# leejeongho3214/LightHand

Hardware: AMD Instinct MI355X
Metric: images/sec/GPU (256×256, bs=64) train+infer; EPE/AUC parity (higher is better)
Workload: dtype bf16; 1 GPU; SimpleBaseline-ResNet50 256x256 training step (fwd + JointsMSELoss + argmax decode + bwd + Adam), batch 64/GPU, 21 joints, random init (seed 9001), hipGraph replay; global_batch=64, parallelism=dp1

## Files before the change

include/lighthand_hip.h:

```cpp
#ifndef LIGHTHAND_HIP_H
#define LIGHTHAND_HIP_H

#include <stddef.h>
#include <stdint.h>

#ifdef __cplusplus
extern "C" {
#endif

typedef enum { LH_F32 = 0, LH_BF16 = 1, LH_F16 = 2 } lh_dtype;

typedef enum {
    LH_OK = 0,
    LH_ERR_ARG = -1,
    LH_ERR_HIP = -2,
    LH_ERR_UNSUPPORTED = -3
} lh_status;

int lh_version(void);
const char* lh_last_error(void);
int lh_dtype_size(int dtype);

int lh_image_to_nhwc4(const float* nchw, void* out, int n, int h, int w, int pad, int wp,
                      int dtype, void* stream);
// ... 74 lines not shown
    const float* mean2;
    const float* invstd2;
    float* partial2;
} lh_bn_bwd_gate;
int lh_igemm_gated_rows(const lh_igemm_desc* d, int dtype, int nterms);
int lh_igemm_gated(const lh_igemm_desc* d, const void* in, const void* wpack, void* out, const void* addend, const void* addend_mask,
                   const lh_bn_bwd_gate* gate, int dtype, void* stream);
int lh_igemm_phases_rows(const lh_igemm_desc* const* descs, int nphase, int dtype);
int lh_igemm_phases(const lh_igemm_desc* const* descs, int nphase, const void* in, const void* const* wpacks,
                    void* out, const void* addend, const void* addend_mask, const float* bias, const float* scale,
                    const float* shift, float* stats, int dtype, void* stream);
typedef struct {
    const void* w;
    size_t w_row_bytes;
    const float* bias;
    float* out;
    int n_out;
} lh_head;
int lh_igemm_phases_head(const lh_igemm_desc* const* descs, int nphase, const void* in, const void* const* wpacks,
                         const float* scale, const float* shift, const lh_head* head, int dtype, void* stream);
int lh_igemm_tile(const lh_igemm_desc* d, int dtype, int* bm, int* bp, int* ring);
int lh_igemm_config(const lh_igemm_desc* d, int dtype, int* cfg5);
int lh_igemm_candidates(const lh_igemm_desc* d, int dtype, int* cfgs, int max);
int lh_wgrad_rowfold(const lh_igemm_desc* d, int rows, const void* x, const void* dy, int dy_pix_stride,
                     int n_out, float* slab, int dtype, void* stream);
int lh_wgrad_tile(const lh_igemm_desc* d, int n_out, int n_in, int dtype, int* bo, int* bi, int* nsplit, int* ring);
int lh_wgrad_candidates(const lh_igemm_desc* d, int n_out, int n_in, int dtype, int* out, int max);
typedef struct {
    const lh_igemm_desc* d; const void* in; const void* wpack; void* out; const void* addend; const void* addend_mask;
    const float* bias; const float* scale; const float* shift; float* stats;
} lh_igemm_call;
int lh_igemm_multi(const lh_igemm_call* calls, int n, int dtype, void* stream);
int lh_igemm_stats_rows(const lh_igemm_desc* d, int dtype);

size_t lh_wgrad_slab_bytes(const lh_igemm_desc* d, int n_out, int n_in, int dtype);
int lh_wgrad(const lh_igemm_desc* d, const void* x, const void* dy, int dy_pix_stride,
             int n_out, int n_in, float* slab, int dtype, void* stream);
int lh_wgrad_reduce(const lh_igemm_desc* d, const float* slab, float* grad, int n_out, int n_in,
                    long so, long si, long sr, long ss, const int* taps_rs, int accumulate,
                    int dtype, void* stream);
size_t lh_wgrad_workspace_bytes(const lh_igemm_desc* d, int n_out, int n_in, int dtype);
typedef struct {
    const lh_igemm_desc* d; int rows; const void* x; const void* dy; int dy_pix_stride, n_out, n_in; void* workspace; float* grad;
    long so, si, sr, ss; const int* taps_rs; int accumulate;
} lh_wgrad_call;
int lh_wgrad_fused_multi(const lh_wgrad_call* calls, int n, int dtype, void* stream);
int lh_wgrad_fused(const lh_igemm_desc* d, int rows, const void* x, const void* dy, int dy_pix_stride, int n_out, int n_in,
                   void* workspace, float* grad, long so, long si, long sr, long ss, const int* taps_rs, int accumulate,
                   int dtype, void* stream);
typedef struct {
    int bo, bi, kps, depth;
    int n_problems, n_fold;
    int n_items, n_fold_items;
    int fold_lds, target_stages, nsplit_max;
    int run_parts;
    size_t off_items, off_fold_args, off_fold_items, table_bytes, workspace_bytes;
} lh_wgrad_table_info;
int lh_wgrad_table_build(const lh_wgrad_call* calls, int n, int dtype, const int* cfg4, int target_stages, void* workspace,
                         void* host_blob, size_t host_bytes, lh_wgrad_table_info* info);
int lh_wgrad_table_run(const void* table, const lh_wgrad_table_info* info, int dtype, void* stream);


int lh_bn_stats(const void* y, int m, int c, float* stats, int* rows_out, int dtype, void* stream);
int lh_bn_stats_rows(int m, int c);
size_t lh_bn_stats_slab_bytes(int rows, int c);
int lh_bn_finalize(const float* stats, int rows, int count, int c, const float* gamma,
// ... 147 lines not shown
```

lighthand_amd/_lib.py:

```python
import ctypes as C
import os

_HERE = os.path.dirname(os.path.abspath(__file__))
LIB_PATH = os.environ.get("LH_LIB_PATH") or os.path.join(_HERE, "liblighthand_hip.so")

LH_F32, LH_BF16, LH_F16 = 0, 1, 2


class LightHandError(RuntimeError):
    pass


class IgemmDesc(C.Structure):
    _fields_ = [("n", C.c_int), ("hi", C.c_int), ("wi", C.c_int), ("in_pix_stride", C.c_int),
                ("k_run", C.c_int), ("ho", C.c_int), ("wo", C.c_int), ("sh", C.c_int), ("sw", C.c_int),
                ("cout", C.c_int), ("OH", C.c_int), ("OW", C.c_int), ("osh", C.c_int), ("osw", C.c_int),
                ("ooh", C.c_int), ("oow", C.c_int), ("out_pix_stride", C.c_int), ("ntaps", C.c_int),
                ("relu", C.c_int), ("dh", C.c_byte * 64), ("dw", C.c_byte * 64), ("cfg", C.c_int * 8)]


class BnFinalizeCall(C.Structure):
    _fields_ = [("stats", C.c_void_p), ("rows", C.c_int), ("count", C.c_int), ("c", C.c_int), ("gamma", C.c_void_p), ("beta", C.c_void_p),
                ("running_mean", C.c_void_p), ("running_var", C.c_void_p), ("num_batches_tracked", C.c_void_p), ("momentum", C.c_float),
                ("eps", C.c_float), ("scale", C.c_void_p), ("shift", C.c_void_p), ("save_mean", C.c_void_p), ("save_invstd", C.c_void_p)]
# ... 69 lines not shown
                ("packs", PackOut * 5)]


_P, _I, _L, _F, _SZ = C.c_void_p, C.c_int, C.c_long, C.c_float, C.c_size_t

SIGNATURES = {
    "lh_version": (_I, []),
    "lh_last_error": (C.c_char_p, []),
    "lh_dtype_size": (_I, [_I]),
    "lh_image_to_nhwc4": (_I, [_P, _P, _I, _I, _I, _I, _I, _I, _P]),
    "lh_image_u8_to_nhwc4": (_I, [_P, _P, _I, _I, _I, _I, _I, _I, _I, C.POINTER(C.c_float), C.POINTER(C.c_float), _I, _P]),
    "lh_image_jitter_workspace_bytes": (_SZ, [_I]),
    "lh_image_u8_jitter_to_nhwc4": (_I, [_P, _P, _I, _I, _I, _I, _I, _I, _I, C.POINTER(C.c_float), C.POINTER(C.c_float), _P, _P, _P, _I, _P]),
    "lh_image_u8_warp_to_nhwc4": (_I, [_P, _P, _I, _I, _I, _I, _I, _I, _I, C.POINTER(C.c_float), C.POINTER(C.c_float), _P, _P, _P, _P, _I, _P]),
    "lh_affine_points": (_I, [_P, _I, _P, _P, _I, _I, _I, _P]),
    "lh_nhwc4_mirror": (_I, [_P, _I, _I, _I, _I, _I, _I, _P]),
    "lh_nhwc_to_nchw_f32": (_I, [_P, _P, _I, _I, _I, _I, _I, _I, _P]),
    "lh_nchw_f32_to_nhwc": (_I, [_P, _P, _I, _I, _I, _I, _I, _I, _P]),
    "lh_pack_weight": (_I, [_P, _P, C.POINTER(_SZ), _I, _I, _L, _L, _L, _L, _I, C.POINTER(_I), _I, _P]),
    "lh_pack_chunk_elems": (_I, []),
    "lh_pack_weights_multi": (_I, [_P, _P, _P, _I, _I, _P]),
    "lh_pack_weights_tiled": (_I, [_P, _P, _P, _P, _I, _I, _I, _P]),
    "lh_igemm": (_I, [C.POINTER(IgemmDesc), _P, _P, _P, _P, _P, _P, _P, _P, _P, _I, _P]),
    "lh_igemm_multi": (_I, [C.POINTER(IgemmCall), _I, _I, _P]),
    "lh_igemm_phases_rows": (_I, [C.POINTER(C.POINTER(IgemmDesc)), _I, _I]),
    "lh_igemm_phases": (_I, [C.POINTER(C.POINTER(IgemmDesc)), _I, _P, C.POINTER(C.c_void_p), _P, _P, _P, _P, _P, _P, _P, _I, _P]),
    "lh_igemm_phases_head": (_I, [C.POINTER(C.POINTER(IgemmDesc)), _I, _P, C.POINTER(C.c_void_p), _P, _P, C.POINTER(Head), _I, _P]),
    "lh_igemm_tile": (_I, [C.POINTER(IgemmDesc), _I, C.POINTER(_I), C.POINTER(_I), C.POINTER(_I)]),
    "lh_igemm_config": (_I, [C.POINTER(IgemmDesc), _I, C.POINTER(_I)]),
    "lh_igemm_candidates": (_I, [C.POINTER(IgemmDesc), _I, C.POINTER(_I), _I]),
    "lh_wgrad_tile": (_I, [C.POINTER(IgemmDesc), _I, _I, _I, C.POINTER(_I), C.POINTER(_I), C.POINTER(_I), C.POINTER(_I)]),
    "lh_wgrad_candidates": (_I, [C.POINTER(IgemmDesc), _I, _I, _I, C.POINTER(_I), _I]),
    "lh_igemm_stats_rows": (_I, [C.POINTER(IgemmDesc), _I]),
    "lh_igemm_gated_rows": (_I, [C.POINTER(IgemmDesc), _I, _I]),
    "lh_igemm_gated": (_I, [C.POINTER(IgemmDesc), _P, _P, _P, _P, _P, C.POINTER(BnBwdGate), _I, _P]),
    "lh_wgrad_slab_bytes": (_SZ, [C.POINTER(IgemmDesc), _I, _I, _I]),
    "lh_wgrad": (_I, [C.POINTER(IgemmDesc), _P, _P, _I, _I, _I, _P, _I, _P]),
    "lh_wgrad_rowfold": (_I, [C.POINTER(IgemmDesc), _I, _P, _P, _I, _I, _P, _I, _P]),
    "lh_wgrad_workspace_bytes": (_SZ, [C.POINTER(IgemmDesc), _I, _I, _I]),
    "lh_wgrad_fused": (_I, [C.POINTER(IgemmDesc), _I, _P, _P, _I, _I, _I, _P, _P, _L, _L, _L, _L, C.POINTER(_I), _I, _I, _P]),
    "lh_wgrad_fused_multi": (_I, [C.POINTER(WgradCall), _I, _I, _P]),
    "lh_wgrad_table_build": (_I, [C.POINTER(WgradCall), _I, _I, C.POINTER(_I), _I, _P, _P, _SZ, C.POINTER(WgradTableInfo)]),
    "lh_wgrad_table_run": (_I, [_P, C.POINTER(WgradTableInfo), _I, _P]),
    "lh_wgrad_reduce": (_I, [C.POINTER(IgemmDesc), _P, _P, _I, _I, _L, _L, _L, _L, C.POINTER(_I), _I, _I, _P]),
    "lh_bn_stats": (_I, [_P, _I, _I, _P, C.POINTER(_I), _I, _P]),
    "lh_bn_stats_rows": (_I, [_I, _I]),
    "lh_bn_stats_slab_bytes": (_SZ, [_I, _I]),
    "lh_bn_finalize": (_I, [_P, _I, _I, _I, _P, _P, _P, _P, _P, _F, _F, _P, _P, _P, _P, _P]),
    "lh_bn_finalize_multi": (_I, [C.POINTER(BnFinalizeCall), _I, _P]),
    "lh_bn_eval_affine": (_I, [_P, _P, _P, _P, _F, _I, _P, _P, _P]),
    "lh_fuse_fwd": (_I, [C.POINTER(FuseDesc), _P, _I, _I, _I, _I, _I, _P]),
    "lh_fuse_fwd_multi": (_I, [C.POINTER(FuseFwdCall), _I, _I, _P]),
    "lh_fuse_bwd_multi": (_I, [C.POINTER(FuseBwdCall), _I, _I, _P]),
    "lh_fuse_bwd_workspace_bytes": (_SZ, [_I, _I, _I, _I]),
    "lh_fuse_bwd": (_I, [C.POINTER(FuseBwdDesc), _I, _I, _I, _I, _P, _I, _P]),
    "lh_stem_pool": (_I, [_P, _I, _I, _I, _P, _P, _P, _P, _P, _I, _I, _I, _I, _P]),
    "lh_bottleneck_infer": (_I, [C.POINTER(BottleneckDesc), _P, _P, _P, _P, _P, _P, _P, _P, _P, _P, _P, _P, _I, _P]),
    "lh_stem_conv_rows": (_I, [_I, _I, _I]),
    "lh_stem_conv": (_I, [_P, _I, _I, _I, _P, _P, _P, _I, _I, _I, _P]),
    "lh_maxpool3x3s2_fwd": (_I, [_P, _P, _P, _I, _I, _I, _I, _I, _P]),
    "lh_maxpool3x3s2_bwd": (_I, [_P, _P, _P, _I, _I, _I, _I, _I, _P]),
    "lh_bn_relu_maxpool3x3s2_fwd": (_I, [_P, _P, _P, _P, _P, _I, _I, _I, _I, _I, _P]),
    "lh_maxpool3x3s2_bwd_gated_rows": (_I, [_I, _I, _I, _I, _I]),
    "lh_maxpool3x3s2_bwd_gated": (_I, [_P, _P, _P, C.POINTER(BnBwdGate), _I, _I, _I, _I, _I, _P]),
    "lh_gaussian_target": (_I, [_P, _I, _P, _I, _P, _I, _I, _I, _P]),
    "lh_gaussian_target_alt": (_I, [_P, _I, _P, _I, _P, _I, _I, _I, _P]),
# ... 65 lines not shown
```

lighthand_amd/csrc/igemm.hip:

```cpp
#include "common.h"
#include <cstring>
#include <algorithm>
#include <stdlib.h>

#include "igemm_args.h"
#include "multi.h"
#include "igemm_ring_cfgs.h"

template <typename T> struct Mma;
template <> struct Mma<bf16> {
    static __device__ __forceinline__ void run(const uint4& a, const uint4& b, f32x4& c) {
        c = __builtin_amdgcn_mfma_f32_16x16x32_bf16(__builtin_bit_cast(bf16x8, a),
                                                   __builtin_bit_cast(bf16x8, b), c, 0, 0, 0);
    }
};
template <> struct Mma<f16> {
    static __device__ __forceinline__ void run(const uint4& a, const uint4& b, f32x4& c) {
        c = __builtin_amdgcn_mfma_f32_16x16x32_f16(__builtin_bit_cast(f16x8, a),
                                                  __builtin_bit_cast(f16x8, b), c, 0, 0, 0);
    }
};
template <> struct Mma<float> {
    static __device__ __forceinline__ void run(const uint4& a, const uint4& b, f32x4& c) {
        const f32x4 fa = __builtin_bit_cast(f32x4, a), fb = __builtin_bit_cast(f32x4, b);
// ... 334 lines not shown
        LH_REQUIRE(gate->x && gate->mean && gate->invstd && gate->partial && (gate->mask || (gate->scale && gate->shift)),
                   "lh_igemm_gated: null pointer in the gate (the sign of the activation comes from scale + shift or from mask)");
        LH_REQUIRE(!bias && !scale && !d->relu && !phases && !head, "lh_igemm_gated: a data gradient carries no bias / affine / ReLU / phases");
        LH_REQUIRE(!gate->mask || d->out_pix_stride == d->cout, "lh_igemm_gated: gate.mask needs a dense output (mask bits index 16-byte chunks)");
        a.gx = (const unsigned char*)gate->x; a.gmean = gate->mean; a.ginv = gate->invstd; a.gscale = gate->scale; a.gshift = gate->shift;
        a.gmask = (const unsigned char*)gate->mask;
        a.stats = gate->partial;
        if (gate->x2) {
            LH_REQUIRE(gate->mask && gate->mean2 && gate->invstd2 && gate->partial2, "lh_igemm_gated: a second BatchNorm term (x2) needs mask, mean2, invstd2, partial2");
            a.gx2 = (const unsigned char*)gate->x2; a.gmean2 = gate->mean2; a.ginv2 = gate->invstd2; a.stats2 = gate->partial2;
        }
    }
    a.n = d->n; a.hi = d->hi; a.wi = d->wi; a.in_pix_stride = d->in_pix_stride; a.k_run = d->k_run;
    a.kspt = (d->k_run * es + 63) / 64;
    a.kpad = (d->k_run * es + 127) / 128 * (128 / es);
    a.ho = d->ho; a.wo = d->wo; a.M = d->n * d->ho * d->wo; a.sh = d->sh; a.sw = d->sw; a.cout = d->cout;
    a.OH = d->OH; a.OW = d->OW; a.osh = d->osh; a.osw = d->osw; a.ooh = d->ooh; a.oow = d->oow;
    a.out_pix_stride = d->out_pix_stride; a.ntaps = d->ntaps; a.relu = d->relu;
    for (int i = 0; i < 64; ++i) { a.dh[i] = d->dh[i]; a.dw[i] = d->dw[i]; }
    int bm, bp;
    RingCfg rc_;
    const bool ring = lh_ring_supported(d, dtype);
    if (ring) {
        const int rc = lh_ring_resolve(d, dtype, &rc_);
        if (rc) return rc;
        bm = rc_.bm; bp = rc_.bp;
    } else {
        pick_tile(d, dtype, &bm, &bp);
    }
    hipStream_t s = (hipStream_t)stream;
    a.tw = 1; a.dh0 = a.dhs = a.dw0 = a.dws = 0;
    a.xcd = 1;
    a.nphase = 1; a.phase_blocks = 0;
    LH_REQUIRE(!(ring && (rc_.depth == 1 || rc_.depth == 100) && (phases || head)), "lh_igemm_phases: the persistent kernels take single launches only");
    if (phases) {
        LH_REQUIRE(ring, "lh_igemm_phases: the form is not supported by the LDS-DMA kernel");
        a.nphase = phases->n;
        a.phase_blocks = ceil_div(a.M, bp) * ceil_div(a.cout, bm);
        for (int i = 0; i < phases->n; ++i) {
            const lh_igemm_desc* q = phases->descs[i];
            a.ph_w[i] = (const unsigned char*)phases->wpacks[i];
            a.ph_ntaps[i] = q->ntaps; a.ph_tw[i] = 1; a.ph_dh0[i] = a.ph_dhs[i] = a.ph_dw0[i] = a.ph_dws[i] = 0;
            if (q->ntaps > 0)
                LH_REQUIRE(lh_tap_grid(q, &a.ph_tw[i], &a.ph_dh0[i], &a.ph_dhs[i], &a.ph_dw0[i], &a.ph_dws[i]) && a.ph_w[i],
                           "lh_igemm_phases: phase %d has an irregular tap list or no weights", i);
            a.ph_ooh[i] = q->ooh; a.ph_oow[i] = q->oow;
            a.ph_row0[i] = i * ceil_div(a.M, bp);
        }
    }
    if (head) {
        LH_REQUIRE(head->w && head->out && head->n_out >= 1 && head->n_out <= 32 && head->w_row_bytes >= d->cout * es,
                   "lh_igemm_phases_head: bad head (1..32 output channels, K-major weight rows)");
        LH_REQUIRE(ring && es == 2 && bm == 256 && bp == 256 && d->cout <= 256 && !addend && !stats,
                   "lh_igemm_phases_head: needs the 256 x 256 tile of the LDS-DMA kernel (cfg), a 16-bit type, <= 256 channels, no addend / statistics");
        a.head_w = (const unsigned char*)head->w; a.head_bias = head->bias; a.head_out = head->out;
        a.head_j = head->n_out; a.head_wstride = (int)head->w_row_bytes;
    }
    if (prep_args) {
        LH_REQUIRE(ring && ((rc_.depth >= 2 && rc_.depth < LH_WIDE_DEPTH) || rc_.depth == 100),
                   "lh_igemm_multi: problem does not run on the LDS-DMA ring kernel or the direct 3x3 kernel (its cfg must name a tiled or the direct configuration)");
        if (rc_.depth == 100) {
            a.pw_cb = (d->cout + 63) / 64;
            a.pw_g = lh_d3_rows(d);
        } else {
            lh_tap_grid(d, &a.tw, &a.dh0, &a.dhs, &a.dw0, &a.dws);
            a.kspt = (d->k_run * es + rc_.kb - 1) / rc_.kb;
// ... 145 lines not shown
```

lighthand_amd/csrc/igemm_args.h:

```cpp
#pragma once
#include "common.h"

struct IgemmArgs {
    const unsigned char* in;
    const unsigned char* w;
    unsigned char* out;
    const unsigned char* addend;
    const unsigned char* addend_mask;
    const unsigned char* zero;
    unsigned char* dump;
    const float* bias;
    const float* scale;
    const float* shift;
    float* stats;
    const unsigned char* gx;
    const float* gmean;
    const float* ginv;
    const float* gscale;
    const float* gshift;
    const unsigned char* gmask;
    const unsigned char* gx2;
    const float* gmean2;
    const float* ginv2;
    float* stats2;
    const unsigned char* head_w;
    const float* head_bias;
    float* head_out;
    int head_j, head_wstride;
    int n, hi, wi, in_pix_stride, k_run, kspt, kpad;
    int ho, wo, M, sh, sw, cout;
    int OH, OW, osh, osw, ooh, oow, out_pix_stride;
    int ntaps, relu;
    int nphase, phase_blocks;
    const unsigned char* ph_w[4];
    int ph_ntaps[4], ph_tw[4], ph_dh0[4], ph_dhs[4], ph_dw0[4], ph_dws[4], ph_ooh[4], ph_oow[4], ph_row0[4];
    int xcd;
    int pw_g, pw_cb;
    int tw, dh0, dhs, dw0, dws;
    signed char dh[64];
    signed char dw[64];
};

struct RingCfg {
    int bm, bp, depth, kb;
};

static inline int lh_pw_lds_bytes(int bm, int kc, int pt, int gate = 0) {
    return bm * kc * 2 + 4 * pt * 16 * (64 * 2 + 8) + (2 + 2 * gate) * bm * 4;
}

static inline void lh_pw_grid(int bm, int kc, int pt, long M, int cout, int occ, int* G, int* CB) {
    const int cb = (cout + bm - 1) / bm;
    const long ntile = (M + pt * 16 - 1) / (pt * 16);
    long g = 256L * occ / cb / 8 * 8;
    const long need = ((ntile + 3) / 4 + 7) / 8 * 8;
    if (g > need) g = need;
    if (g < 8) g = 8;
    *G = (int)g;
    *CB = cb;
}


bool lh_ring_supported(const lh_igemm_desc* d, int dtype);
bool lh_tap_grid(const lh_igemm_desc* d, int* tw, int* dh0, int* dhs, int* dw0, int* dws);
int lh_ring_resolve(const lh_igemm_desc* d, int dtype, RingCfg* out);
void lh_ring_default_cfg(const lh_igemm_desc* d, int dtype, RingCfg* out);
int lh_ring_candidates(const lh_igemm_desc* d, int dtype, int* out, int max);
int lh_igemm_ring_launch(const IgemmArgs& a, const RingCfg& c, int dtype, hipStream_t s);
template <typename A> struct LhMulti;
int lh_igemm_ring_multi_launch(LhMulti<IgemmArgs>& m, const RingCfg& c, int dtype, hipStream_t s);
bool lh_pw_supported(const lh_igemm_desc* d, int dtype);
// ... 5 lines not shown
```

lighthand_amd/csrc/igemm_epilogue.h:

```cpp
#pragma once
#include "common.h"
#include "igemm_args.h"

#ifndef LH_ABL
#define LH_ABL 0
#endif

template <typename T, int BM, int BP, bool HEAD> constexpr int lh_epi_lds_bytes() {
    return BP * (BM * (int)sizeof(T) + 8) + (HEAD ? 32 * (BM * (int)sizeof(T) + 16) : 0) + 3 * BM * 4;
}

template <int BM, int NT>
__device__ __forceinline__ void igemm_epilogue_consts(const IgemmArgs& p, float* cst, int c0, int tid) {
    const int cmax = p.cout - 1;
    for (int c = tid; c < BM; c += NT) {
        const int gc = c0 + c, gk = gc < cmax ? gc : cmax;
        const bool ok = gc < p.cout;
        const float b = p.bias ? p.bias[gk] : 0.f, sc = p.scale ? p.scale[gk] : 1.f, sh = p.scale ? p.shift[gk] : 0.f;
        float bv = (p.bias && ok) ? b : 0.f, sv = 1.f;
        if (p.scale) {
            sv = ok ? sc : 1.f;
            bv = bv * sv + (ok ? sh : 0.f);
        }
        cst[c] = sv;
// ... 37 lines not shown
            b4 = *reinterpret_cast<const float4*>(cst + BM + col);
        }
        const float sv[4] = {s4.x, s4.y, s4.z, s4.w}, bv[4] = {b4.x, b4.y, b4.z, b4.w};
#pragma unroll
        for (int j = 0; j < PT; ++j) {
            const int pr = wp * TP + j * 16 + pl;
            T* dst = reinterpret_cast<T*>(smem + pr * RS + col * ES);
            if constexpr (ES == 4) {
                reinterpret_cast<float2*>(dst)[0] = float2{acc[i][j][0] * sv[0] + bv[0], acc[i][j][1] * sv[1] + bv[1]};
                reinterpret_cast<float2*>(dst)[1] = float2{acc[i][j][2] * sv[2] + bv[2], acc[i][j][3] * sv[3] + bv[3]};
            } else {
                union { uint2 u; T e[4]; } pk;
#pragma unroll
                for (int r = 0; r < 4; ++r) pk.e[r] = from_f<T>(acc[i][j][r] * sv[r] + bv[r]);
                *reinterpret_cast<uint2*>(dst) = pk.u;
            }
        }
    }
    __syncthreads();

    constexpr int CH = BM * ES / 16;
    constexpr int NT = 64 * WC * WP;
    constexpr int RPP = NT / CH;
    const int chunk = tid % CH, r0 = tid / CH;
    const int col0 = cblk * BM + chunk * EPC;
    const bool col_ok = col0 < p.cout;
    float s1[EPC], s2[EPC];
#pragma unroll
    for (int e = 0; e < EPC; ++e) s1[e] = s2[e] = 0.f;

    const bool dense = p.osh == 1 && p.osw == 1 && p.OH == p.ho && p.OW == p.wo && ooh == 0 && oow == 0;
    int m = pblk * BP + r0;
    int pn = 0, pa = 0, pb = 0;
    const int qa = RPP / p.wo, step_b = RPP - qa * p.wo, step_n = qa / p.ho, step_a = qa - step_n * p.ho;
    if (!dense) {
        pn = m / hw;
        const int rem = m - pn * hw;
        pa = rem / p.wo;
        pb = rem - pa * p.wo;
    }
    constexpr int NR = BP / RPP;
    static_assert(BP % RPP == 0, "rows per thread");
    int opx[NR];
    uint4 ad[NR];
    uint4 xd[NR];
    unsigned mbits[NR];
    unsigned gbits[NR];
    float gmean[EPC], ginv[EPC], gsc[EPC], gsh[EPC];
    if (p.gx) {
#pragma unroll
        for (int e = 0; e < EPC; ++e) {
            const int gk = col0 + e < p.cout ? col0 + e : p.cout - 1;
            gmean[e] = p.gmean[gk]; ginv[e] = p.ginv[gk];
            gsc[e] = p.gmask ? 0.f : p.gscale[gk]; gsh[e] = p.gmask ? 0.f : p.gshift[gk];
        }
    }
#pragma unroll
    for (int k = 0; k < NR; ++k, m += RPP) {
        int opix = m;
        if (!dense) {
            opix = (pn * p.OH + pa * p.osh + ooh) * p.OW + pb * p.osw + oow;
            pb += step_b; pa += step_a; pn += step_n;
            if (pb >= p.wo) { pb -= p.wo; ++pa; }
            if (pa >= p.ho) { pa -= p.ho; ++pn; }
        }
        opx[k] = (m < p.M && col_ok) ? opix : -1;
        ad[k] = uint4{0u, 0u, 0u, 0u};
        mbits[k] = 0xffu;
        if (p.addend) {
            const bool ok = opx[k] >= 0;
            const long eoff = (long)((unsigned long)(unsigned)(ok ? opx[k] : 0) * (unsigned)p.out_pix_stride) + col0;
// ... 122 lines not shown
            *reinterpret_cast<uint4*>(hw_lds + row * HS + ch * 16) = v;
        }
    }
    __syncthreads();
    constexpr int PW = BP / NW;
    constexpr int NPT = PW / 16;
    f32x4 hacc[2][NPT];
#pragma unroll
    for (int a = 0; a < 2; ++a)
#pragma unroll
        for (int b = 0; b < NPT; ++b) hacc[a][b] = f32x4{0.f, 0.f, 0.f, 0.f};
    const int l15 = lane & 15, kg = lane >> 4;
#pragma unroll 2
    for (int ks = 0; ks < BM / 32; ++ks) {
        uint4 fa[2], fb[NPT];
#pragma unroll
        for (int a = 0; a < 2; ++a) fa[a] = *reinterpret_cast<const uint4*>(hw_lds + (a * 16 + l15) * HS + (ks * 32 + kg * 8) * ES);
#pragma unroll
        for (int b = 0; b < NPT; ++b) {
            const unsigned char* src = smem + (wave * PW + b * 16 + l15) * RS + (ks * 32 + kg * 8) * ES;
            const uint2 lo = *reinterpret_cast<const uint2*>(src), hi = *reinterpret_cast<const uint2*>(src + 8);
            fb[b] = uint4{lo.x, lo.y, hi.x, hi.y};
        }
#pragma unroll
        for (int a = 0; a < 2; ++a)
#pragma unroll
            for (int b = 0; b < NPT; ++b) MMA::run(fa[a], fb[b], hacc[a][b]);
    }
    const long plane = (long)p.OH * p.OW;
#pragma unroll
    for (int b = 0; b < NPT; ++b) {
        const int m = pblk * BP + wave * PW + b * 16 + l15;
        if (m >= p.M) continue;
        const int n = m / hw, rem = m - n * hw;
        const int ya = rem / p.wo, xb = rem - ya * p.wo;
        const long opix = (long)(ya * p.osh + ooh) * p.OW + xb * p.osw + oow;
#pragma unroll
        for (int a = 0; a < 2; ++a)
#pragma unroll
            for (int r = 0; r < 4; ++r) {
                const int j = a * 16 + kg * 4 + r;
                if (j < p.head_j) p.head_out[((long)n * p.head_j + j) * plane + opix] = hacc[a][b][r] + (p.head_bias ? p.head_bias[j] : 0.f);
            }
    }
}
```

lighthand_amd/csrc/igemm_ring.hip:

```cpp
#include "common.h"

#include "igemm_args.h"
#include "multi.h"
#include "igemm_ring_cfgs.h"
#include "igemm_pw_cfgs.h"
#include <stdlib.h>
#include <cstdlib>
#include <mutex>

int lh_ring_launch_bf16_big(const IgemmArgs& a, const RingCfg& c, hipStream_t s);
int lh_ring_launch_bf16_mid(const IgemmArgs& a, const RingCfg& c, hipStream_t s);
int lh_ring_launch_bf16_small(const IgemmArgs& a, const RingCfg& c, hipStream_t s);
int lh_ring_launch_f16_big(const IgemmArgs& a, const RingCfg& c, hipStream_t s);
int lh_ring_launch_f16_mid(const IgemmArgs& a, const RingCfg& c, hipStream_t s);
int lh_ring_launch_f16_small(const IgemmArgs& a, const RingCfg& c, hipStream_t s);
int lh_ring_launch_bf16_dense(const IgemmArgs& a, const RingCfg& c, hipStream_t s);
int lh_ring_launch_f16_dense(const IgemmArgs& a, const RingCfg& c, hipStream_t s);
int lh_ring_launch_f32(const IgemmArgs& a, const RingCfg& c, hipStream_t s);
int lh_ring_multi_launch_bf16(const LhMulti<IgemmArgs>& m, const RingCfg& c, hipStream_t s);
int lh_ring_multi_launch_f16(const LhMulti<IgemmArgs>& m, const RingCfg& c, hipStream_t s);
int lh_pw_launch_bf16(const IgemmArgs& a, const RingCfg& c, hipStream_t s);
int lh_pw_launch_f16(const IgemmArgs& a, const RingCfg& c, hipStream_t s);
int lh_d3_launch_bf16(const IgemmArgs& a, const RingCfg& c, hipStream_t s);
int lh_d3_launch_f16(const IgemmArgs& a, const RingCfg& c, hipStream_t s);
// ... 242 lines not shown

static const unsigned char* zero_page() {
    static std::mutex mu;
    static const unsigned char* ptr[64] = {nullptr};
    int dev = 0;
    if (hipGetDevice(&dev) != hipSuccess || dev < 0 || dev >= 64) return nullptr;
    std::lock_guard<std::mutex> lock(mu);
    if (!ptr[dev]) {
        void* q = nullptr;
        if (hipGetSymbolAddress(&q, HIP_SYMBOL(lh_zero_page)) != hipSuccess) return nullptr;
        ptr[dev] = (const unsigned char*)q;
    }
    return ptr[dev];
}

static int lh_ring_offsets_fit(const IgemmArgs& a, int bm, int bp, int es) {
    const long ipix = (long)a.in_pix_stride * es, img = (long)a.hi * a.wi * ipix;
    const long hw = (long)a.ho * a.wo > 0 ? (long)a.ho * a.wo : 1;
    long reach = (bp / hw + 2) * img;
    for (int ph = 0; ph < (a.nphase > 1 ? a.nphase : 1); ++ph) {
        const int ntaps = a.nphase > 1 ? a.ph_ntaps[ph] : a.ntaps, tw = a.nphase > 1 ? a.ph_tw[ph] : a.tw;
        const int dh0 = a.nphase > 1 ? a.ph_dh0[ph] : a.dh0, dhs = a.nphase > 1 ? a.ph_dhs[ph] : a.dhs;
        const int dw0 = a.nphase > 1 ? a.ph_dw0[ph] : a.dw0, dws = a.nphase > 1 ? a.ph_dws[ph] : a.dws;
        const int th = tw > 0 ? (ntaps + tw - 1) / tw : 1;
        const long shift = ((long)(std::abs(dh0) + std::abs(dhs) * th) * a.wi + std::abs(dw0) + std::abs(dws) * tw) * ipix;
        LH_REQUIRE(reach + 2 * shift + (long)a.k_run * es + 256 < (1L << 31) && (long)bm * ntaps * a.kpad * es < (1L << 31),
                   "igemm_ring: a %d-pixel tile of this launch reaches %ld bytes of input (%d x %d pixels of %ld bytes per image, tap window %ld) "
                   "or %ld bytes of weights: more than the 2 GiB a workgroup's buffer descriptor addresses",
                   bp, reach + 2 * shift, a.hi, a.wi, ipix, shift, (long)bm * ntaps * a.kpad * es);
    }
    return LH_OK;
}

const unsigned char* lh_ring_zero_page() { return zero_page(); }
unsigned char* lh_ring_dump_page() { return dump_page(); }

int lh_igemm_ring_launch(const IgemmArgs& a0, const RingCfg& c, int dtype, hipStream_t s) {
    IgemmArgs a = a0;
    a.zero = zero_page();
    a.dump = dump_page();
    if (!a.zero || !a.dump) {
        lh_set_error("igemm_ring: cannot resolve the zero page on this device");
        return LH_ERR_HIP;
    }
    int rc = 1;
    if (c.depth == 100) {
        if (dtype == LH_BF16) rc = lh_d3_launch_bf16(a, c, s);
        else if (dtype == LH_F16) rc = lh_d3_launch_f16(a, c, s);
        if (rc == 1) {
            lh_set_error("conv3x3_direct: no kernel for %d input channels, dtype %d", c.kb, dtype);
            return LH_ERR_UNSUPPORTED;
        }
        return rc;
    }
    if (c.depth == 1) {
        if (dtype == LH_BF16) rc = lh_pw_launch_bf16(a, c, s);
        else if (dtype == LH_F16) rc = lh_pw_launch_f16(a, c, s);
        if (rc == 1) {
            lh_set_error("igemm_pw: no kernel for panel %d x K %d, %d pixels per wave, dtype %d", c.bm, c.kb, c.bp, dtype);
            return LH_ERR_UNSUPPORTED;
        }
        return rc;
    }
    if (int e = lh_ring_offsets_fit(a, c.bm, c.bp, dtype == LH_F32 ? 4 : 2)) return e;
    switch (dtype) {
        case LH_BF16:
            rc = lh_ring_launch_bf16_big(a, c, s);
            if (rc == 1) rc = lh_ring_launch_bf16_mid(a, c, s);
            if (rc == 1) rc = lh_ring_launch_bf16_small(a, c, s);
            if (rc == 1) rc = lh_ring_launch_bf16_dense(a, c, s);
            break;
        case LH_F16:
            rc = lh_ring_launch_f16_big(a, c, s);
            if (rc == 1) rc = lh_ring_launch_f16_mid(a, c, s);
            if (rc == 1) rc = lh_ring_launch_f16_small(a, c, s);
            if (rc == 1) rc = lh_ring_launch_f16_dense(a, c, s);
            break;
        case LH_F32:
            rc = lh_ring_launch_f32(a, c, s);
            break;
        default:
            lh_set_error("igemm_ring: unsupported dtype %d", dtype);
            return LH_ERR_ARG;
    }
    if (rc == 1) {
        lh_set_error("igemm_ring: no kernel for tile %dx%d depth %d kb %d dtype %d", c.bm, c.bp, c.depth, c.kb, dtype);
        return LH_ERR_UNSUPPORTED;
    }
    return rc;
}

int lh_igemm_ring_multi_launch(LhMulti<IgemmArgs>& m, const RingCfg& c, int dtype, hipStream_t s) {
    const unsigned char* z = zero_page();
    if (!z) {
        lh_set_error("igemm_ring_multi: cannot resolve the zero page on this device");
        return LH_ERR_HIP;
    }
    for (int i = 0; i < m.n; ++i) { m.a[i].zero = z; m.a[i].dump = dump_page(); }
    for (int i = 0; i < m.n; ++i)
        if (int e = lh_ring_offsets_fit(m.a[i], c.bm, c.bp, 2)) return e;
    int rc = 1;
    if (dtype == LH_BF16) rc = lh_ring_multi_launch_bf16(m, c, s);
    else if (dtype == LH_F16) rc = lh_ring_multi_launch_f16(m, c, s);
    if (rc == 1) {
        lh_set_error("igemm_ring_multi: no multi-problem kernel for tile %dx%d depth %d kb %d dtype %d (4-wave tiles, 16-bit types)",
                     c.bm, c.bp, c.depth, c.kb, dtype);
        return LH_ERR_UNSUPPORTED;
    }
    return rc;
}
```

lighthand_amd/csrc/igemm_ring_kernel.h:

```cpp
#pragma once
#include "common.h"
#include "igemm_args.h"
#include "igemm_epilogue.h"
#include "multi.h"

#include <type_traits>

template <typename T> struct MmaR;
template <> struct MmaR<bf16> {
    static __device__ __forceinline__ void run(const uint4& a, const uint4& b, f32x4& c) {
        c = __builtin_amdgcn_mfma_f32_16x16x32_bf16(__builtin_bit_cast(bf16x8, a), __builtin_bit_cast(bf16x8, b), c, 0, 0, 0);
    }
};
template <> struct MmaR<f16> {
    static __device__ __forceinline__ void run(const uint4& a, const uint4& b, f32x4& c) {
        c = __builtin_amdgcn_mfma_f32_16x16x32_f16(__builtin_bit_cast(f16x8, a), __builtin_bit_cast(f16x8, b), c, 0, 0, 0);
    }
};
template <> struct MmaR<float> {
    static __device__ __forceinline__ void run(const uint4& a, const uint4& b, f32x4& c) {
        const f32x4 fa = __builtin_bit_cast(f32x4, a), fb = __builtin_bit_cast(f32x4, b);
        c = __builtin_amdgcn_mfma_f32_16x16x4f32(fa[0], fb[0], c, 0, 0, 0);
        c = __builtin_amdgcn_mfma_f32_16x16x4f32(fa[1], fb[1], c, 0, 0, 0);
        c = __builtin_amdgcn_mfma_f32_16x16x4f32(fa[2], fb[2], c, 0, 0, 0);
        c = __builtin_amdgcn_mfma_f32_16x16x4f32(fa[3], fb[3], c, 0, 0, 0);
    }
};

#ifndef LH_ABL
#define LH_ABL 0
#endif

typedef __attribute__((address_space(3))) void* lds_void_p;
typedef const __attribute__((address_space(1))) void* gbl_void_p;

template <int I> using ic = std::integral_constant<int, I>;
template <int B, int E, typename F> __device__ __forceinline__ void static_for(F&& f) {
    if constexpr (B < E) {
        f(ic<B>{});
        static_for<B + 1, E>(f);
    }
}

template <int L, int MAXS> __device__ __forceinline__ void wait_stages(int stages) {
    static_assert(MAXS * L <= 63, "vmcnt is a 6-bit counter");
    if constexpr (MAXS == 0) {
        asm volatile("s_waitcnt vmcnt(0)" ::: "memory");
    } else {
        if (stages >= MAXS) asm volatile("s_waitcnt vmcnt(%0)" ::"n"(MAXS * L) : "memory");
        else wait_stages<L, MAXS - 1>(stages);
    }
}

template <typename T, int BM, int BP, int WC, int WP, int D, int KB>
__device__ __forceinline__ void igemm_ring_body(const IgemmArgs& p, unsigned char* smem, const int bid, const int nblk) {
#if defined(__HIP_DEVICE_COMPILE__)
    constexpr int ES = sizeof(T);
    constexpr int EPC = 16 / ES;
    constexpr int KSTEP = KB / ES;
    constexpr int TC = BM / WC, TP = BP / WP;
    constexpr int CT = TC / 16, PT = TP / 16;
    constexpr int STAGE = (BM + BP) * KB;
    constexpr int H = KB / 64;
    constexpr int SL = KB / 16;
    constexpr int RPI = 64 / SL;
    constexpr int GB = 16 * KB;
    constexpr int NWAVE = WC * WP;
    constexpr int NW = BM / 16 * H / NWAVE, NX = BP / 16 * H / NWAVE;
    constexpr int L = NW + NX;
    constexpr int KSUB = KB / 64;
    constexpr int NR = PT + CT;
    static_assert((NWAVE == 4 || NWAVE == 8) && D >= 2 && D <= 10 && (KB == 64 || KB == 128) && NW >= 1 && NX >= 1, "bad configuration");

    const int tid = threadIdx.x, lane = tid & 63;
    const int wave = __builtin_amdgcn_readfirstlane(tid >> 6);
    const int wc = wave / WP, wp = wave % WP;
    const int CB = (p.cout + BM - 1) / BM;
    int w = p.xcd ? lh_xcd_remap(bid, nblk) : bid;
    const unsigned char* wgt = p.w;
    int ntaps = p.ntaps, tw = p.tw, dh0 = p.dh0, dhs = p.dhs, dw0 = p.dw0, dws = p.dws, ooh = p.ooh, oow = p.oow;
    float* stats = p.stats;
    if (p.nphase > 1) {
        const int ph = w % p.nphase;
        w /= p.nphase;
        wgt = p.ph_w[ph]; ntaps = p.ph_ntaps[ph]; tw = p.ph_tw[ph];
        dh0 = p.ph_dh0[ph]; dhs = p.ph_dhs[ph]; dw0 = p.ph_dw0[ph]; dws = p.ph_dws[ph];
        ooh = p.ph_ooh[ph]; oow = p.ph_oow[ph];
        if (stats) stats += (long)p.ph_row0[ph] * 2 * p.cout;
    }
    const int pblk = w / CB, cblk = w - pblk * CB;
    const int hw = p.ho * p.wo;

    constexpr unsigned OOR = 0x80000000u;
    const int th = (ntaps + tw - 1) / tw;
    const long ipix = (long)p.in_pix_stride * ES;
    const long shift = ((long)((dh0 < 0 ? -dh0 : dh0) + (dhs < 0 ? -dhs : dhs) * th) * p.wi + (dw0 < 0 ? -dw0 : dw0) + (dws < 0 ? -dws : dws) * tw) * ipix;
    const long img_bytes = (long)p.hi * p.wi * ipix;
    const int m_first = pblk * BP < p.M ? pblk * BP : p.M - 1;
    const int n_first = m_first / hw;
    const long in_off = (long)n_first * img_bytes - shift;
    const long in_rec = (long)p.n * img_bytes - in_off + 16;
    const auto rs_in = __builtin_amdgcn_make_buffer_rsrc((void*)(p.in + in_off), 0, (int)(in_rec < 0x7fffffffL ? in_rec : 0x7fffffffL), 0x00020000);
    const long kpad = p.kpad;
    const long w_off = (long)cblk * BM * ntaps * kpad * ES;
    const auto rs_w = __builtin_amdgcn_make_buffer_rsrc((void*)(wgt + w_off), 0, (int)((long)BM * ntaps * kpad * ES), 0x00020000);
    unsigned pvoff[NX], cvoff[NX];
    unsigned tmask[NX];
    int klim[NX];
    const bool kfull = p.k_run % KSTEP == 0;
#pragma unroll
    for (int j = 0; j < NX; ++j) {
        const int q = NWAVE * j + wave;
        const int g = q / H, lrow = (q % H) * RPI + lane / SL;
        const int c = (lane % SL) ^ ((lrow / (16 / SL)) & (SL - 1));
        const int row = g * 16 + lrow;
        const int m = pblk * BP + row;
        const bool ok = m < p.M;
        const int mm = ok ? m : m_first;
        const int n = mm / hw, rem = mm - n * hw;
        const int a = rem / p.wo, b = rem - a * p.wo;
        const int ih0 = a * p.sh, iw0 = b * p.sw;
        pvoff[j] = (unsigned)(((long)((n - n_first) * p.hi * p.wi + ih0 * p.wi + iw0) * p.in_pix_stride + c * EPC) * ES);
        klim[j] = p.k_run - c * EPC;
        unsigned tm = 0;
        int t = 0;
        for (int ti = 0, dh = dh0; ti * tw < ntaps; ++ti, dh += dhs)
            for (int tjj = 0, dw = dw0; tjj < tw; ++tjj, dw += dws, ++t)
                if (ok && (unsigned)(ih0 + dh) < (unsigned)p.hi && (unsigned)(iw0 + dw) < (unsigned)p.wi) tm |= 1u << t;
        tmask[j] = tm;
        cvoff[j] = ((tm & 1u) != 0 && klim[j] > 0) ? pvoff[j] : OOR;
    }
    unsigned wvoff[NW];
#pragma unroll
    for (int j = 0; j < NW; ++j) {
        const int q = NWAVE * j + wave;
        const int g = q / H, lrow = (q % H) * RPI + lane / SL;
        const int c = (lane % SL) ^ ((lrow / (16 / SL)) & (SL - 1));
        const int row = g * 16 + lrow;
        wvoff[j] = (unsigned)(((long)row * ntaps * kpad + c * EPC) * ES);
    }
    const unsigned lds_base = (unsigned)(size_t)(__attribute__((address_space(3))) unsigned char*)smem;

    int itap = 0, ikc = 0, tj = 0, cdh = dh0, cdw = dw0;
    int issued = 0, islot = 0;
    int woff = 0;
    auto issue = [&]() {
        unsigned char* st = smem + islot * STAGE;
#pragma unroll
        for (int j = 0; j < NW; ++j) {
            const int q = NWAVE * j + wave;
            if (!(LH_ABL & 4))
                __builtin_amdgcn_raw_ptr_buffer_load_lds(rs_w, (lds_void_p)(st + (q / H) * GB + (q % H) * 1024), 16, wvoff[j], woff, 0, 0);
        }
        const int kbase = ikc * KSTEP;
        const int soff = (int)(shift + ((long)(cdh * p.wi + cdw) * p.in_pix_stride + kbase) * ES);
#pragma unroll
        for (int j = 0; j < NX; ++j) {
            const int q = NWAVE * j + wave;
            if (!(LH_ABL & 4))
                __builtin_amdgcn_raw_ptr_buffer_load_lds(rs_in, (lds_void_p)(st + BM * KB + (q / H) * GB + (q % H) * 1024), 16, cvoff[j], soff, 0, 0);
        }
        ++issued;
        if (++islot == D) islot = 0;
        woff += KB;
        bool retap = false;
        if (++ikc == p.kspt) {
            ikc = 0; ++itap;
            woff = (int)((long)itap * kpad * ES);
            cdw += dws;
            if (++tj == tw) { tj = 0; cdw = dw0; cdh += dhs; }
            retap = true;
        }
        if (retap || !kfull) {
            const int kb2 = ikc * KSTEP;
#pragma unroll
            for (int j = 0; j < NX; ++j) cvoff[j] = (((tmask[j] >> itap) & 1u) != 0 && kb2 < klim[j]) ? pvoff[j] : OOR;
        }
    };

    f32x4 acc[CT][PT];
#pragma unroll
    for (int i = 0; i < CT; ++i)
#pragma unroll
        for (int j = 0; j < PT; ++j) acc[i][j] = f32x4{0.f, 0.f, 0.f, 0.f};

    const int S = ntaps * p.kspt;
#pragma unroll
    for (int s = 0; s < D - 1; ++s)
        if (issued < S) issue();

    unsigned offA[KSUB], offB[KSUB];
#pragma unroll
    for (int kk = 0; kk < KSUB; ++kk) {
        const int c = 4 * kk + (lane >> 4), r = lane & 15;
        const unsigned foff = r * KB + ((c ^ ((r / (16 / SL)) & (SL - 1))) << 4);
        offA[kk] = lds_base + wc * CT * GB + foff;
        offB[kk] = lds_base + BM * KB + wp * PT * GB + foff;
    }
    auto rd = [](auto Rc, uint4& dst, unsigned base_a, unsigned base_b) {
        constexpr int r = decltype(Rc)::value;
        if constexpr ((LH_ABL & 2) != 0) { dst = uint4{base_a, base_b, base_a, base_b}; return; }
        if constexpr (r < PT) asm volatile("ds_read_b128 %0, %1 offset:%2" : "=v"(dst) : "v"(base_b), "n"(r * GB));
        else asm volatile("ds_read_b128 %0, %1 offset:%2" : "=v"(dst) : "v"(base_a), "n"((r - PT) * GB));
    };
    auto step_at = [&](const unsigned ca, const unsigned cb) {
        uint4 F[NR];
        static_for<0, NR>([&](auto r) { rd(r, F[decltype(r)::value], ca, cb); });
        static_for<0, CT>([&](auto Ic) {
            constexpr int i = decltype(Ic)::value;
            __builtin_amdgcn_sched_barrier(0);
            asm volatile("s_waitcnt lgkmcnt(%0)" ::"n"(CT - 1 - i) : "memory");
            __builtin_amdgcn_sched_barrier(0);
#pragma unroll
            for (int j = 0; j < PT; ++j)
                if (!(LH_ABL & 1)) MmaR<T>::run(F[PT + i], F[j], acc[i][j]);
        });
    };
    auto step = [&](auto KKc, unsigned so) { step_at(offA[decltype(KKc)::value] + so, offB[decltype(KKc)::value] + so); };

    const bool late = NWAVE == 8 && KSUB == 2 && wave >= NWAVE / 2;
    int cslot = 0;
    for (int s = 0; s < S; ++s) {
        wait_stages<L, D - 2>(issued - 1 - s);
        __builtin_amdgcn_s_barrier();
        const unsigned so = cslot * STAGE;
        if (++cslot == D) cslot = 0;
        if (!late && issued < S) issue();
        step(ic<0>{}, so);
        if constexpr (KSUB == 2) {
            if (late && issued < S) issue();
            step(ic<1>{}, so);
        }
    }
    if constexpr (BM == 256 && BP == 256 && sizeof(T) == 2) {
        if (p.head_w) {
            igemm_epilogue_head<T, BM, BP, WC, WP, MmaR<T>>(p, smem, acc, pblk, tid, lane, wave, wc, wp, hw, ooh, oow);
            return;
        }
    }
    igemm_epilogue<T, BM, BP, WC, WP>(p, smem, acc, pblk, cblk, tid, lane, wc, wp, hw, ooh, oow, stats);
#endif
}

template <int BM, int BP, int WC, int WP> constexpr int ring_waves_per_simd() { return 2; }

template <typename T, int BM, int BP, int WC, int WP, int D, int KB>
__global__ __launch_bounds__(64 * WC * WP, (ring_waves_per_simd<BM, BP, WC, WP>())) void igemm_ring_kernel(const IgemmArgs p) {
    extern __shared__ __attribute__((aligned(16))) unsigned char smem[];
    igemm_ring_body<T, BM, BP, WC, WP, D, KB>(p, smem, blockIdx.x, gridDim.x);
}

template <typename T, int BM, int BP, int WC, int WP, int D, int KB>
__global__ __launch_bounds__(64 * WC * WP, 2) void igemm_ring_multi_kernel(const LhMulti<IgemmArgs> m) {
    extern __shared__ __attribute__((aligned(16))) unsigned char smem[];
    int bid, nblk;
    const int i = lh_multi_pick(m, bid, nblk);
    igemm_ring_body<T, BM, BP, WC, WP, D, KB>(m.a[i], smem, bid, nblk);
}

template <typename T, int BM, int BP, int WC, int WP, int D, int KB>
static int launch_ring(const IgemmArgs& a, hipStream_t s) {
    constexpr int ES = sizeof(T);
    constexpr int ring = D * (BM + BP) * KB;
    constexpr int epi = lh_epi_lds_bytes<T, BM, BP, (BM == 256 && BP == 256 && ES == 2)>();
    constexpr int lds = ring > epi ? ring : epi;
    static_assert(lds <= 160 * 1024, "LDS budget");
// ... 34 lines not shown
```

Measured before the change: 7532 images/s.

## Issue weight prologue loads early and replace integer divides with magic multiply

Host-computed magic multiplier/shift pairs replace per-thread integer divisions by ho*wo, wo and nphase in the ring kernel prologue and epilogues. The weight-tile LDS-DMA loads for the pipeline prologue are now issued before the input-offset and tap-mask setup, so their latency overlaps that address arithmetic. The tap-mask construction is restructured into separate column and row masks. New ablation bits and a full vmcnt wait after the prologue when D>2 are added; that wait may stall the first stage.

```diff
diff --git a/include/lighthand_hip.h b/include/lighthand_hip.h
--- a/include/lighthand_hip.h
+++ b/include/lighthand_hip.h
@@ -130,6 +130,7 @@
 } lh_igemm_call;
 int lh_igemm_multi(const lh_igemm_call* calls, int n, int dtype, void* stream);
 int lh_igemm_stats_rows(const lh_igemm_desc* d, int dtype);
+int lh_magic_u32(unsigned divisor, unsigned* mul, unsigned* shift);
 
 size_t lh_wgrad_slab_bytes(const lh_igemm_desc* d, int n_out, int n_in, int dtype);
 int lh_wgrad(const lh_igemm_desc* d, const void* x, const void* dy, int dy_pix_stride,
diff --git a/lighthand_amd/_lib.py b/lighthand_amd/_lib.py
--- a/lighthand_amd/_lib.py
+++ b/lighthand_amd/_lib.py
@@ -125,6 +125,7 @@
     "lh_wgrad_tile": (_I, [C.POINTER(IgemmDesc), _I, _I, _I, C.POINTER(_I), C.POINTER(_I), C.POINTER(_I), C.POINTER(_I)]),
     "lh_wgrad_candidates": (_I, [C.POINTER(IgemmDesc), _I, _I, _I, C.POINTER(_I), _I]),
     "lh_igemm_stats_rows": (_I, [C.POINTER(IgemmDesc), _I]),
+    "lh_magic_u32": (_I, [C.c_uint, C.POINTER(C.c_uint), C.POINTER(C.c_uint)]),
     "lh_igemm_gated_rows": (_I, [C.POINTER(IgemmDesc), _I, _I]),
     "lh_igemm_gated": (_I, [C.POINTER(IgemmDesc), _P, _P, _P, _P, _P, C.POINTER(BnBwdGate), _I, _P]),
     "lh_wgrad_slab_bytes": (_SZ, [C.POINTER(IgemmDesc), _I, _I, _I]),
diff --git a/lighthand_amd/csrc/igemm.hip b/lighthand_amd/csrc/igemm.hip
--- a/lighthand_amd/csrc/igemm.hip
+++ b/lighthand_amd/csrc/igemm.hip
@@ -390,6 +390,7 @@
     a.tw = 1; a.dh0 = a.dhs = a.dw0 = a.dws = 0;
     a.xcd = 1;
     a.nphase = 1; a.phase_blocks = 0;
+    a.mg_hw = a.mg_wo = a.mg_nphase = LhMagic{0u, 0u};
     LH_REQUIRE(!(ring && (rc_.depth == 1 || rc_.depth == 100) && (phases || head)), "lh_igemm_phases: the persistent kernels take single launches only");
     if (phases) {
         LH_REQUIRE(ring, "lh_igemm_phases: the form is not supported by the LDS-DMA kernel");
diff --git a/lighthand_amd/csrc/igemm_args.h b/lighthand_amd/csrc/igemm_args.h
--- a/lighthand_amd/csrc/igemm_args.h
+++ b/lighthand_amd/csrc/igemm_args.h
@@ -1,5 +1,18 @@
 #pragma once
 #include "common.h"
+
+struct LhMagic {
+    unsigned mul, shift;
+};
+static inline LhMagic lh_magic(unsigned d) {
+    unsigned l = 0;
+    while (l < 31 && (1u << l) < d) ++l;
+    const unsigned long long num = 1ull << (31 + l);
+    return LhMagic{(unsigned)((num + d - 1) / d), l};
+}
+#if defined(__HIPCC__)
+__device__ __forceinline__ int lh_magic_div(int n, const LhMagic& m) { return (int)(__umulhi((unsigned)n << 1, m.mul) >> m.shift); }
+#endif
 
 struct IgemmArgs {
     const unsigned char* in;
@@ -37,6 +50,7 @@
     int xcd;
     int pw_g, pw_cb;
     int tw, dh0, dhs, dw0, dws;
+    LhMagic mg_hw, mg_wo, mg_nphase;
     signed char dh[64];
     signed char dw[64];
 };
diff --git a/lighthand_amd/csrc/igemm_epilogue.h b/lighthand_amd/csrc/igemm_epilogue.h
--- a/lighthand_amd/csrc/igemm_epilogue.h
+++ b/lighthand_amd/csrc/igemm_epilogue.h
@@ -93,11 +93,13 @@
     const bool dense = p.osh == 1 && p.osw == 1 && p.OH == p.ho && p.OW == p.wo && ooh == 0 && oow == 0;
     int m = pblk * BP + r0;
     int pn = 0, pa = 0, pb = 0;
-    const int qa = RPP / p.wo, step_b = RPP - qa * p.wo, step_n = qa / p.ho, step_a = qa - step_n * p.ho;
+    int step_b = 0, step_n = 0, step_a = 0;
     if (!dense) {
-        pn = m / hw;
+        const int qa = lh_magic_div(RPP, p.mg_wo);
+        step_b = RPP - qa * p.wo; step_n = qa / p.ho; step_a = qa - step_n * p.ho;
+        pn = lh_magic_div(m, p.mg_hw);
         const int rem = m - pn * hw;
-        pa = rem / p.wo;
+        pa = lh_magic_div(rem, p.mg_wo);
         pb = rem - pa * p.wo;
     }
     constexpr int NR = BP / RPP;
@@ -286,8 +288,8 @@
     for (int b = 0; b < NPT; ++b) {
         const int m = pblk * BP + wave * PW + b * 16 + l15;
         if (m >= p.M) continue;
-        const int n = m / hw, rem = m - n * hw;
-        const int ya = rem / p.wo, xb = rem - ya * p.wo;
+        const int n = lh_magic_div(m, p.mg_hw), rem = m - n * hw;
+        const int ya = lh_magic_div(rem, p.mg_wo), xb = rem - ya * p.wo;
         const long opix = (long)(ya * p.osh + ooh) * p.OW + xb * p.osw + oow;
 #pragma unroll
         for (int a = 0; a < 2; ++a)
diff --git a/lighthand_amd/csrc/igemm_ring.hip b/lighthand_amd/csrc/igemm_ring.hip
--- a/lighthand_amd/csrc/igemm_ring.hip
+++ b/lighthand_amd/csrc/igemm_ring.hip
@@ -298,6 +298,20 @@
     return LH_OK;
 }
 
+static void lh_ring_fill_magic(IgemmArgs& a) {
+    a.mg_hw = lh_magic((unsigned)(a.ho * a.wo));
+    a.mg_wo = lh_magic((unsigned)a.wo);
+    a.mg_nphase = lh_magic((unsigned)(a.nphase > 1 ? a.nphase : 1));
+}
+
+extern "C" int lh_magic_u32(unsigned divisor, unsigned* mul, unsigned* shift) {
+    LH_REQUIRE(mul && shift, "lh_magic_u32: null pointer");
+    LH_REQUIRE(divisor >= 1 && divisor <= 0x80000000u, "lh_magic_u32: divisor %u outside 1 .. 2^31", divisor);
+    const LhMagic m = lh_magic(divisor);
+    *mul = m.mul; *shift = m.shift;
+    return LH_OK;
+}
+
 const unsigned char* lh_ring_zero_page() { return zero_page(); }
 unsigned char* lh_ring_dump_page() { return dump_page(); }
 
@@ -329,6 +343,7 @@
         return rc;
     }
     if (int e = lh_ring_offsets_fit(a, c.bm, c.bp, dtype == LH_F32 ? 4 : 2)) return e;
+    lh_ring_fill_magic(a);
     switch (dtype) {
         case LH_BF16:
             rc = lh_ring_launch_bf16_big(a, c, s);
@@ -362,7 +377,7 @@
         lh_set_error("igemm_ring_multi: cannot resolve the zero page on this device");
         return LH_ERR_HIP;
     }
-    for (int i = 0; i < m.n; ++i) { m.a[i].zero = z; m.a[i].dump = dump_page(); }
+    for (int i = 0; i < m.n; ++i) { m.a[i].zero = z; m.a[i].dump = dump_page(); lh_ring_fill_magic(m.a[i]); }
     for (int i = 0; i < m.n; ++i)
         if (int e = lh_ring_offsets_fit(m.a[i], c.bm, c.bp, 2)) return e;
     int rc = 1;
diff --git a/lighthand_amd/csrc/igemm_ring_kernel.h b/lighthand_amd/csrc/igemm_ring_kernel.h
--- a/lighthand_amd/csrc/igemm_ring_kernel.h
+++ b/lighthand_amd/csrc/igemm_ring_kernel.h
@@ -30,6 +30,7 @@
 #ifndef LH_ABL
 #define LH_ABL 0
 #endif
+static_assert(!(LH_ABL & 64) || (LH_ABL & 4), "LH_ABL 64 makes up offsets: only without the loads (bit 4)");
 
 typedef __attribute__((address_space(3))) void* lds_void_p;
 typedef const __attribute__((address_space(1))) void* gbl_void_p;
@@ -79,10 +80,11 @@
     int w = p.xcd ? lh_xcd_remap(bid, nblk) : bid;
     const unsigned char* wgt = p.w;
     int ntaps = p.ntaps, tw = p.tw, dh0 = p.dh0, dhs = p.dhs, dw0 = p.dw0, dws = p.dws, ooh = p.ooh, oow = p.oow;
-    float* stats = p.stats;
+    float* stats = (LH_ABL & 128) ? nullptr : p.stats;
     if (p.nphase > 1) {
-        const int ph = w % p.nphase;
-        w /= p.nphase;
+        const int wq = lh_magic_div(w, p.mg_nphase);
+        const int ph = w - wq * p.nphase;
+        w = wq;
         wgt = p.ph_w[ph]; ntaps = p.ph_ntaps[ph]; tw = p.ph_tw[ph];
         dh0 = p.ph_dh0[ph]; dhs = p.ph_dhs[ph]; dw0 = p.ph_dw0[ph]; dws = p.ph_dws[ph];
         ooh = p.ph_ooh[ph]; oow = p.ph_oow[ph];
@@ -90,46 +92,12 @@
     }
     const int pblk = w / CB, cblk = w - pblk * CB;
     const int hw = p.ho * p.wo;
+    const int S = ntaps * p.kspt;
 
     constexpr unsigned OOR = 0x80000000u;
-    const int th = (ntaps + tw - 1) / tw;
-    const long ipix = (long)p.in_pix_stride * ES;
-    const long shift = ((long)((dh0 < 0 ? -dh0 : dh0) + (dhs < 0 ? -dhs : dhs) * th) * p.wi + (dw0 < 0 ? -dw0 : dw0) + (dws < 0 ? -dws : dws) * tw) * ipix;
-    const long img_bytes = (long)p.hi * p.wi * ipix;
-    const int m_first = pblk * BP < p.M ? pblk * BP : p.M - 1;
-    const int n_first = m_first / hw;
-    const long in_off = (long)n_first * img_bytes - shift;
-    const long in_rec = (long)p.n * img_bytes - in_off + 16;
-    const auto rs_in = __builtin_amdgcn_make_buffer_rsrc((void*)(p.in + in_off), 0, (int)(in_rec < 0x7fffffffL ? in_rec : 0x7fffffffL), 0x00020000);
     const long kpad = p.kpad;
     const long w_off = (long)cblk * BM * ntaps * kpad * ES;
     const auto rs_w = __builtin_amdgcn_make_buffer_rsrc((void*)(wgt + w_off), 0, (int)((long)BM * ntaps * kpad * ES), 0x00020000);
-    unsigned pvoff[NX], cvoff[NX];
-    unsigned tmask[NX];
-    int klim[NX];
-    const bool kfull = p.k_run % KSTEP == 0;
-#pragma unroll
-    for (int j = 0; j < NX; ++j) {
-        const int q = NWAVE * j + wave;
-        const int g = q / H, lrow = (q % H) * RPI + lane / SL;
-        const int c = (lane % SL) ^ ((lrow / (16 / SL)) & (SL - 1));
-        const int row = g * 16 + lrow;
-        const int m = pblk * BP + row;
-        const bool ok = m < p.M;
-        const int mm = ok ? m : m_first;
-        const int n = mm / hw, rem = mm - n * hw;
-        const int a = rem / p.wo, b = rem - a * p.wo;
-        const int ih0 = a * p.sh, iw0 = b * p.sw;
-        pvoff[j] = (unsigned)(((long)((n - n_first) * p.hi * p.wi + ih0 * p.wi + iw0) * p.in_pix_stride + c * EPC) * ES);
-        klim[j] = p.k_run - c * EPC;
-        unsigned tm = 0;
-        int t = 0;
-        for (int ti = 0, dh = dh0; ti * tw < ntaps; ++ti, dh += dhs)
-            for (int tjj = 0, dw = dw0; tjj < tw; ++tjj, dw += dws, ++t)
-                if (ok && (unsigned)(ih0 + dh) < (unsigned)p.hi && (unsigned)(iw0 + dw) < (unsigned)p.wi) tm |= 1u << t;
-        tmask[j] = tm;
-        cvoff[j] = ((tm & 1u) != 0 && klim[j] > 0) ? pvoff[j] : OOR;
-    }
     unsigned wvoff[NW];
 #pragma unroll
     for (int j = 0; j < NW; ++j) {
@@ -140,18 +108,78 @@
         wvoff[j] = (unsigned)(((long)row * ntaps * kpad + c * EPC) * ES);
     }
     const unsigned lds_base = (unsigned)(size_t)(__attribute__((address_space(3))) unsigned char*)smem;
+    unsigned sink = 0;
+    auto issue_w = [&](unsigned char* st, const int woff_) {
+#pragma unroll
+        for (int j = 0; j < NW; ++j) {
+            const int q = NWAVE * j + wave;
+            if (!(LH_ABL & 4))
+                __builtin_amdgcn_raw_ptr_buffer_load_lds(rs_w, (lds_void_p)(st + (q / H) * GB + (q % H) * 1024), 16, wvoff[j], woff_, 0, 0);
+            else sink ^= wvoff[j] + (unsigned)woff_;
+        }
+    };
+    {
+        int pt = 0, pk = 0, po = 0;
+#pragma unroll
+        for (int s = 0; s < D - 1; ++s)
+            if (s < S) {
+                issue_w(smem + s * STAGE, po);
+                po += KB;
+                if (++pk == p.kspt) { pk = 0; ++pt; po = (int)((long)pt * kpad * ES); }
+            }
+    }
+
+    const int th = (ntaps + tw - 1) / tw;
+    const long ipix = (long)p.in_pix_stride * ES;
+    const long shift = ((long)((dh0 < 0 ? -dh0 : dh0) + (dhs < 0 ? -dhs : dhs) * th) * p.wi + (dw0 < 0 ? -dw0 : dw0) + (dws < 0 ? -dws : dws) * tw) * ipix;
+    const long img_bytes = (long)p.hi * p.wi * ipix;
+    const int m_first = pblk * BP < p.M ? pblk * BP : p.M - 1;
+    const int n_first = lh_magic_div(m_first, p.mg_hw);
+    const long in_off = (long)n_first * img_bytes - shift;
+    const long in_rec = (long)p.n * img_bytes - in_off + 16;
+    const auto rs_in = __builtin_amdgcn_make_buffer_rsrc((void*)(p.in + in_off), 0, (int)(in_rec < 0x7fffffffL ? in_rec : 0x7fffffffL), 0x00020000);
+    unsigned pvoff[NX], cvoff[NX];
+    unsigned tmask[NX];
+    int klim[NX];
+    const bool kfull = p.k_run % KSTEP == 0;
+    const unsigned tap_bits = ntaps >= 32 ? ~0u : (1u << ntaps) - 1u;
+#pragma unroll
+    for (int j = 0; j < NX; ++j) {
+        const int q = NWAVE * j + wave;
+        const int g = q / H, lrow = (q % H) * RPI + lane / SL;
+        const int c = (lane % SL) ^ ((lrow / (16 / SL)) & (SL - 1));
+        if constexpr ((LH_ABL & 64) != 0) {
+            pvoff[j] = (unsigned)(lane * 16 + j * 1024);
+            klim[j] = p.k_run;
+            tmask[j] = ~0u;
+            cvoff[j] = pvoff[j];
+            continue;
+        }
+        const int row = g * 16 + lrow;
+        const int m = pblk * BP + row;
+        const bool ok = m < p.M;
+        const int mm = ok ? m : m_first;
+        const int n = lh_magic_div(mm, p.mg_hw), rem = mm - n * hw;
+        const int a = lh_magic_div(rem, p.mg_wo), b = rem - a * p.wo;
+        const int ih0 = a * p.sh, iw0 = b * p.sw;
+        pvoff[j] = (unsigned)(((long)((n - n_first) * p.hi * p.wi + ih0 * p.wi + iw0) * p.in_pix_stride + c * EPC) * ES);
+        klim[j] = p.k_run - c * EPC;
+        unsigned cm = 0, tm = 0;
+        for (int tjj = 0, dw = dw0; tjj < tw; ++tjj, dw += dws)
+            if ((unsigned)(iw0 + dw) < (unsigned)p.wi) cm |= 1u << tjj;
+        for (int ti = 0, dh = dh0; ti * tw < ntaps; ++ti, dh += dhs)
+            if ((unsigned)(ih0 + dh) < (unsigned)p.hi) tm |= cm << (ti * tw);
+        tm = ok ? tm & tap_bits : 0u;
+        tmask[j] = tm;
+        cvoff[j] = ((tm & 1u) != 0 && klim[j] > 0) ? pvoff[j] : OOR;
+    }
 
     int itap = 0, ikc = 0, tj = 0, cdh = dh0, cdw = dw0;
     int issued = 0, islot = 0;
     int woff = 0;
-    auto issue = [&]() {
+    auto issue = [&](auto WW) {
         unsigned char* st = smem + islot * STAGE;
-#pragma unroll
-        for (int j = 0; j < NW; ++j) {
-            const int q = NWAVE * j + wave;
-            if (!(LH_ABL & 4))
-                __builtin_amdgcn_raw_ptr_buffer_load_lds(rs_w, (lds_void_p)(st + (q / H) * GB + (q % H) * 1024), 16, wvoff[j], woff, 0, 0);
-        }
+        if constexpr (decltype(WW)::value != 0) issue_w(st, woff);
         const int kbase = ikc * KSTEP;
         const int soff = (int)(shift + ((long)(cdh * p.wi + cdw) * p.in_pix_stride + kbase) * ES);
 #pragma unroll
@@ -159,6 +187,7 @@
             const int q = NWAVE * j + wave;
             if (!(LH_ABL & 4))
                 __builtin_amdgcn_raw_ptr_buffer_load_lds(rs_in, (lds_void_p)(st + BM * KB + (q / H) * GB + (q % H) * 1024), 16, cvoff[j], soff, 0, 0);
+            else sink ^= cvoff[j] + (unsigned)soff;
         }
         ++issued;
         if (++islot == D) islot = 0;
@@ -184,10 +213,10 @@
 #pragma unroll
         for (int j = 0; j < PT; ++j) acc[i][j] = f32x4{0.f, 0.f, 0.f, 0.f};
 
-    const int S = ntaps * p.kspt;
 #pragma unroll
     for (int s = 0; s < D - 1; ++s)
-        if (issued < S) issue();
+        if (issued < S) issue(ic<0>{});
+    if constexpr (D > 2) asm volatile("s_waitcnt vmcnt(0)" ::: "memory");
 
     unsigned offA[KSUB], offB[KSUB];
 #pragma unroll
@@ -225,13 +254,14 @@
         __builtin_amdgcn_s_barrier();
         const unsigned so = cslot * STAGE;
         if (++cslot == D) cslot = 0;
-        if (!late && issued < S) issue();
+        if (!late && issued < S) issue(ic<1>{});
         step(ic<0>{}, so);
         if constexpr (KSUB == 2) {
-            if (late && issued < S) issue();
+            if (late && issued < S) issue(ic<1>{});
             step(ic<1>{}, so);
         }
     }
+    if constexpr ((LH_ABL & 4) != 0) acc[0][0][0] += __uint_as_float(sink & 0x007fffffu);
     if constexpr (BM == 256 && BP == 256 && sizeof(T) == 2) {
         if (p.head_w) {
             igemm_epilogue_head<T, BM, BP, WC, WP, MmaR<T>>(p, smem, acc, pblk, tid, lane, wave, wc, wp, hw, ooh, oow);
```

Result: no change. 7556 images/s (median of 6 runs) (+0.3%).
